# jzr99/Geo4D

Measured on AMD Instinct MI355X. Metric: denoised latent frames/sec (16x320x512, 50-step DDIM), higher is better.
Workload: dtype bf16x3m

## Files before the change

### geo4d_amd/_lib.py

```python
import ctypes as C
import os

import torch

_HERE = os.path.dirname(os.path.abspath(__file__))
LIB_PATH = os.environ.get("GEO4D_HIP_LIB") or os.path.join(_HERE, "csrc", "libgeo4d_hip.so")
ABI_VERSION = 9

F32, BF16, F16, BF16X3, F16X2 = 0, 1, 2, 3, 4


class Geo4DNativeError(RuntimeError):
    pass


class ConvGemm(C.Structure):
    _fields_ = [
        ("A", C.c_void_p), ("W", C.c_void_p), ("O", C.c_void_p),
        ("bias", C.c_void_p), ("rowbias", C.c_void_p), ("R", C.c_void_p),
        ("zeros", C.c_void_p), ("workspace", C.c_void_p), ("workspace_bytes", C.c_size_t),
        ("lda", C.c_long), ("ldw", C.c_long), ("ldo", C.c_long), ("ldr", C.c_long), ("ldrb", C.c_long),
        ("a_bs", C.c_long), ("w_bs", C.c_long), ("o_bs", C.c_long), ("r_bs", C.c_long),
        ("M", C.c_int), ("N", C.c_int), ("K", C.c_int), ("batch", C.c_int),
        ("Cin", C.c_int),
# ... 14 lines not shown
        ("ldx", C.c_long), ("ldy", C.c_long),
        ("F", C.c_int), ("HW", C.c_int), ("C", C.c_int), ("groups", C.c_int), ("frames_per_stat", C.c_int),
        ("act", C.c_int), ("dtype", C.c_int), ("eps", C.c_float), ("colsum", C.c_void_p), ("split_out", C.c_int), ("colsum_rows", C.c_int),
        ("sat_count", C.c_void_p),
    ]


class Attention(C.Structure):
    _fields_ = [
        ("q", C.c_void_p), ("o", C.c_void_p),
        ("k", C.c_void_p * 2), ("vt", C.c_void_p * 2), ("zeros", C.c_void_p),
        ("ldq", C.c_long), ("ldo", C.c_long), ("ldk", C.c_long * 2), ("ldvt", C.c_long * 2), ("vt_bs", C.c_long * 2),
        ("Nk", C.c_int * 2), ("kv_div", C.c_int * 2),
        ("B", C.c_int), ("H", C.c_int), ("Nq", C.c_int), ("nseg", C.c_int), ("head_dim", C.c_int), ("dtype", C.c_int),
        ("scale", C.c_float), ("split_out", C.c_int), ("variant", C.c_int), ("qkv_split", C.c_int),
    ]


class Align(C.Structure):
    _fields_ = [
        ("pred", C.c_void_p), ("conf", C.c_void_p), ("logdepth", C.c_void_p), ("cams", C.c_void_p), ("slot_trf", C.c_void_p),
        ("slot_ptr", C.c_void_p), ("slot_idx", C.c_void_p),
        ("grad_logdepth", C.c_void_p), ("img_sums", C.c_void_p), ("slot_sums", C.c_void_p),
        ("workspace", C.c_void_p), ("workspace_bytes", C.c_size_t),
        ("img_part", C.c_void_p), ("slot_part", C.c_void_p),
        ("invdepth", C.c_void_p), ("slot_st", C.c_void_p),
        ("n_imgs", C.c_int), ("n_slots", C.c_int), ("H", C.c_int), ("W", C.c_int), ("chunk_pixels", C.c_int), ("max_slots_per_image", C.c_int),
        ("conf_clamp", C.c_float), ("inv_area", C.c_float), ("depth_weight", C.c_float),
    ]


class AlignSmall(C.Structure):
    _fields_ = [
        ("im_poses", C.c_void_p), ("im_focals", C.c_void_p), ("pw_poses", C.c_void_p), ("cams", C.c_void_p), ("slot_trf", C.c_void_p),
        ("img_sums", C.c_void_p), ("slot_sums", C.c_void_p), ("group_ptr", C.c_void_p), ("group_entries", C.c_void_p), ("group_sums", C.c_void_p),
        ("scale_terms", C.c_void_p),
        ("grad_im_poses", C.c_void_p), ("grad_im_focals", C.c_void_p), ("grad_pw_poses", C.c_void_p), ("grad_s_depth", C.c_void_p),
        ("grad_t_depth", C.c_void_p), ("loss", C.c_void_p),
        ("slot_st", C.c_void_p), ("s_depth", C.c_void_p), ("t_depth", C.c_void_p), ("depth_ok", C.c_void_p),
        ("traj", C.c_void_p), ("traj_align", C.c_void_p), ("traj_valid", C.c_void_p), ("slot_img", C.c_void_p), ("img_slot_ptr", C.c_void_p),
        ("img_slot_idx", C.c_void_p), ("grad_traj", C.c_void_p),
        ("n_imgs", C.c_int), ("n_groups", C.c_int), ("n_slots", C.c_int), ("slots_per_group", C.c_int), ("n_listed_slots", C.c_int),
        ("n_focals", C.c_int), ("norm_pw_scale", C.c_int),
        ("focal_break", C.c_float), ("base_scale", C.c_float), ("ppx", C.c_float), ("ppy", C.c_float), ("smooth_weight", C.c_float),
        ("translation_weight", C.c_float), ("traj_weight", C.c_float),
    ]


SIGNATURES = {
    "geo4d_conv_gemm": (C.c_int, [C.POINTER(ConvGemm), C.c_void_p]),
    "geo4d_conv_gemm_colsum_rows": (C.c_int, [C.POINTER(ConvGemm)]),
    "geo4d_groupnorm_workspace": (C.c_size_t, [C.c_int, C.c_int, C.c_int, C.c_int]),
    "geo4d_groupnorm": (C.c_int, [C.POINTER(GroupNorm), C.c_void_p]),
    "geo4d_layernorm": (C.c_int, [C.c_void_p, C.c_long, C.c_void_p, C.c_long, C.c_int, C.c_int, C.c_float, C.c_void_p,
                                  C.c_void_p, C.c_int, C.c_void_p]),
    "geo4d_layernorm_split": (C.c_int, [C.c_void_p, C.c_long, C.c_void_p, C.c_long, C.c_int, C.c_int, C.c_float, C.c_void_p,
                                        C.c_void_p, C.c_int, C.c_void_p, C.c_void_p]),
    "geo4d_softmax_rows": (C.c_int, [C.c_void_p, C.c_long, C.c_void_p, C.c_long, C.c_long, C.c_int, C.c_float, C.c_int,
                                     C.c_void_p]),
    "geo4d_softmax_rows_causal": (C.c_int, [C.c_void_p, C.c_long, C.c_void_p, C.c_long, C.c_long, C.c_int, C.c_float, C.c_int,
                                            C.c_int, C.c_void_p]),
    "geo4d_attention": (C.c_int, [C.POINTER(Attention), C.c_void_p]),
    "geo4d_temporal_attention": (C.c_int, [C.c_void_p, C.c_long, C.c_void_p, C.c_long, C.c_void_p, C.c_long, C.c_void_p,
                                           C.c_long, C.c_int, C.c_int, C.c_int, C.c_int, C.c_int, C.c_float, C.c_int,
                                           C.c_void_p]),
    "geo4d_temporal_attention2": (C.c_int, [C.c_void_p, C.c_long, C.c_void_p, C.c_long, C.c_void_p, C.c_long, C.c_void_p,
                                            C.c_long, C.c_int, C.c_int, C.c_int, C.c_int, C.c_int, C.c_float, C.c_int,
                                            C.c_int, C.c_void_p]),
    "geo4d_tokens_from_ncthw": (C.c_int, [C.c_void_p, C.c_int, C.c_void_p, C.c_int, C.c_void_p, C.c_int, C.c_int, C.c_int,
                                          C.c_int, C.c_int, C.c_void_p]),
    "geo4d_cast_rows_f16": (C.c_int, [C.c_void_p, C.c_long, C.c_void_p, C.c_long, C.c_long, C.c_int, C.c_void_p, C.c_void_p]),
    "geo4d_split_rows_bf16": (C.c_int, [C.c_void_p, C.c_long, C.c_void_p, C.c_long, C.c_long, C.c_int, C.c_void_p]),
    "geo4d_concat_channels": (C.c_int, [C.c_void_p, C.c_long, C.c_int, C.c_void_p, C.c_long, C.c_int, C.c_void_p, C.c_long,
                                        C.c_long, C.c_int, C.c_void_p]),
    "geo4d_timestep_embedding": (C.c_int, [C.c_void_p, C.c_void_p, C.c_void_p, C.c_int, C.c_int, C.c_void_p]),
    "geo4d_linear_small": (C.c_int, [C.c_void_p, C.c_long, C.c_void_p, C.c_long, C.c_void_p, C.c_void_p, C.c_long,
                                     C.c_void_p, C.c_long, C.c_int, C.c_int, C.c_int, C.c_int, C.c_int, C.c_void_p]),
    "geo4d_ddim_step": (C.c_int, [C.c_void_p, C.c_void_p, C.c_void_p, C.c_void_p, C.c_void_p, C.c_void_p, C.c_long,
                                  C.c_void_p]),
    "geo4d_cfg_combine_workspace": (C.c_size_t, [C.c_int]),
    "geo4d_cfg_combine": (C.c_int, [C.c_void_p, C.c_void_p, C.c_void_p, C.c_void_p, C.c_int, C.c_long, C.c_float, C.c_float,
                                    C.c_float, C.c_void_p, C.c_size_t, C.c_void_p]),
    "geo4d_embed_tokens": (C.c_int, [C.c_void_p, C.c_void_p, C.c_void_p, C.c_void_p, C.c_long, C.c_long, C.c_int, C.c_int, C.c_int,
                                     C.c_int, C.c_void_p]),
    "geo4d_advance_index": (C.c_int, [C.c_void_p, C.c_int, C.c_void_p]),
    "geo4d_gather_timestep": (C.c_int, [C.c_void_p, C.c_void_p, C.c_void_p, C.c_int, C.c_void_p]),
    "geo4d_plucker_cameras_workspace": (C.c_size_t, [C.c_int, C.c_int, C.c_int]),
    "geo4d_plucker_cameras": (C.c_int, [C.c_void_p, C.c_void_p, C.c_long, C.c_long, C.c_int, C.c_int, C.c_int, C.c_void_p,
                                        C.c_size_t, C.c_void_p, C.c_void_p]),
    "geo4d_align_workspace": (C.c_size_t, [C.c_int, C.c_int, C.c_int, C.c_int, C.c_int]),
    "geo4d_align_residual": (C.c_int, [C.POINTER(Align), C.c_void_p]),
    "geo4d_adam_step": (C.c_int, [C.c_void_p, C.c_void_p, C.c_void_p, C.c_void_p, C.c_long, C.c_float, C.c_float, C.c_float, C.c_float,
                                  C.c_int, C.c_void_p]),
    "geo4d_adam_step_dev": (C.c_int, [C.c_void_p, C.c_void_p, C.c_void_p, C.c_void_p, C.c_long, C.c_void_p, C.c_float, C.c_float, C.c_float,
                                      C.c_void_p]),
    "geo4d_lad_workspace": (C.c_size_t, [C.c_int, C.c_long]),
    "geo4d_lad_target": (C.c_int, [C.c_void_p, C.c_void_p, C.c_void_p, C.c_int, C.c_int, C.c_void_p]),
    "geo4d_lower_median": (C.c_int, [C.c_void_p, C.c_int, C.c_long, C.c_void_p, C.c_void_p, C.c_size_t, C.c_void_p]),
    "geo4d_lad_fit": (C.c_int, [C.c_void_p, C.c_void_p, C.c_int, C.c_long, C.c_void_p, C.c_float, C.c_int, C.c_float, C.c_void_p, C.c_void_p,
                                C.c_void_p, C.c_size_t, C.c_void_p]),
    "geo4d_lad_delta": (C.c_int, [C.c_void_p, C.c_void_p, C.c_void_p, C.c_void_p, C.c_int, C.c_long, C.c_float, C.c_float, C.c_float,
                                  C.c_void_p, C.c_void_p]),
    "geo4d_bicubic_resize": (C.c_int, [C.c_void_p, C.c_void_p, C.c_int, C.c_int, C.c_int, C.c_int, C.c_int, C.c_void_p]),
    "geo4d_masked_select_workspace": (C.c_size_t, [C.c_long]),
    "geo4d_masked_select": (C.c_int, [C.c_void_p, C.c_void_p, C.c_long, C.c_float, C.c_void_p, C.c_float, C.c_float, C.c_void_p, C.c_void_p,
                                      C.c_void_p, C.c_void_p, C.c_size_t, C.c_void_p]),
# ... 56 lines not shown
```

### geo4d_amd/csrc/norm.hip

```cpp
#include <type_traits>
#include "common.h"
#include "geo4d_hip.h"

namespace {

__host__ __device__ inline int gn_rows_per_chunk(int HW, int F) {
    long r = ((long)HW * F + 1023) / 1024;
    r = (r + 3) / 4 * 4;
    if (r < 4) r = 4;
    if (r > 1024) r = 1024;
    return (int)r;
}

template <typename T>
__device__ __forceinline__ void gn_partial_body(char* smem, const T* __restrict__ x, long ldx, int HW, int C, int G,
                                                int R, int nchunk, float* __restrict__ part, int chunk, int f) {
    constexpr int EPC = Elem<T>::EPC;
    float* stage = (float*)smem;
    float* chs = stage + 256 * 2 * EPC;
    float* chq = chs + C;
    const int tid = threadIdx.x;
    const int CPR = C / EPC;
    const int TC = CPR < 256 ? CPR : 256;
    const int TR = 256 / TC;
// ... 50 lines not shown
        float m2 = qq - ss * mean;
        if (m2 < 0.f) m2 = 0.f;
        float* o = part + (((long)f * nchunk + chunk) * G + tid) * 3;
        o[0] = n; o[1] = mean; o[2] = m2;
    }
}
template <typename T>
__global__ __launch_bounds__(256) void gn_partial_kernel(const T* __restrict__ x, long ldx, int HW, int C, int G,
                                                         int R, int nchunk, float* __restrict__ part) {
    extern __shared__ __attribute__((aligned(16))) char smem[];
    gn_partial_body<T>(smem, x, ldx, HW, C, G, R, nchunk, part, blockIdx.x, blockIdx.y);
}

__device__ __forceinline__ void chan_merge(float& n, float& mean, float& m2, float nb, float mb, float qb) {
    if (nb > 0.f) {
        const float nn = n + nb;
        const float d = mb - mean;
        const float w = nb / nn;
        mean += d * w;
        m2 += qb + d * d * n * w;
        n = nn;
    }
}
__device__ __forceinline__ f32x2 gn_merge_unit(const float* __restrict__ part, int total, int stat, int grp, int G, float eps, int lane) {
    float n = 0.f, mean = 0.f, m2 = 0.f;
    for (int i = lane; i < total; i += 64) {
        const float* pp = part + (((long)stat * total + i) * G + grp) * 3;
        chan_merge(n, mean, m2, pp[0], pp[1], pp[2]);
    }
#pragma unroll
    for (int o = 1; o < 64; o <<= 1) {
        const float nb = __shfl_xor(n, o), mb = __shfl_xor(mean, o), qb = __shfl_xor(m2, o);
        float n0 = n, a0 = mean, q0 = m2, n1 = nb, a1 = mb, q1 = qb;
        if (lane & o) { n0 = nb; a0 = mb; q0 = qb; n1 = n; a1 = mean; q1 = m2; }
        chan_merge(n0, a0, q0, n1, a1, q1);
        n = n0; mean = a0; m2 = q0;
    }
    return f32x2{mean, 1.0f / sqrtf(m2 / n + eps)};
}
__global__ __launch_bounds__(256) void gn_finalize_kernel(const float* __restrict__ part, int nchunk, int fps, int G,
                                                          float eps, float* __restrict__ stats, int nstat) {
    const int lane = threadIdx.x & 63;
    const int unit = blockIdx.x * 4 + (threadIdx.x >> 6);
    if (unit >= nstat * G) return;
    const int stat = unit / G, grp = unit - stat * G;
    const f32x2 r = gn_merge_unit(part, fps * nchunk, stat, grp, G, eps, lane);
    if (lane == 0) {
        stats[((long)stat * G + grp) * 2 + 0] = r[0];
        stats[((long)stat * G + grp) * 2 + 1] = r[1];
    }
}

__global__ __launch_bounds__(256) void gn_finalize_cols_kernel(const float* __restrict__ colsum, int blocks_per_stat, int C, int G, float eps,
                                                               float* __restrict__ stats, int nstat, int rows) {
    __shared__ double red[4][2];
    const int tid = threadIdx.x, lane = tid & 63, wave = tid >> 6;
    const int unit = blockIdx.x;
    const int stat = unit / G, grp = unit - stat * G;
    const int cpg = C / G;
    double s = 0.0, q = 0.0;
    const int total = blocks_per_stat * cpg;
    for (int i = tid; i < total; i += 256) {
        const int rb = i / cpg, c = grp * cpg + (i - rb * cpg);
        const f32x2 sq = *(const f32x2*)(colsum + (((long)stat * blocks_per_stat + rb) * C + c) * 2);
        s += (double)sq[0];
        q += (double)sq[1];
    }
#pragma unroll
    for (int o = 1; o < 64; o <<= 1) {
        s += __shfl_xor(s, o);
        q += __shfl_xor(q, o);
    }
    if (lane == 0) { red[wave][0] = s; red[wave][1] = q; }
    __syncthreads();
    if (tid == 0) {
        s = ((red[0][0] + red[1][0]) + red[2][0]) + red[3][0];
        q = ((red[0][1] + red[1][1]) + red[2][1]) + red[3][1];
        const double n = (double)blocks_per_stat * rows * cpg;
        const double mean = s / n;
        double var = q / n - mean * mean;
        if (var < 0.0) var = 0.0;
        stats[((long)stat * G + grp) * 2 + 0] = (float)mean;
        stats[((long)stat * G + grp) * 2 + 1] = (float)(1.0 / sqrt(var + (double)eps));
    }
}

template <typename T, int SPLIT>
__device__ __forceinline__ void gn_apply_body(const T* __restrict__ x, long ldx, T* __restrict__ y, long ldy,
                                              int HW, int C, int G, int R, const float* st, const float* __restrict__ gamma,
                                              const float* __restrict__ beta, int act, int chunk, int f, unsigned long long* sat) {
    constexpr int EPC = Elem<T>::EPC;
    const int tid = threadIdx.x;
    const int CPR = C / EPC;
    const int TC = CPR < 256 ? CPR : 256;
    const int TR = 256 / TC;
    const int tc = tid % TC, tr = tid / TC;
    if (tr >= TR) return;
    const int row0 = chunk * R;
    const int rows = min(R, HW - row0);
    const int cpg = C / G;
    const T* xb = x + ((long)f * HW + row0) * ldx;
    T* yb = y + ((long)f * HW + row0) * ldy;
    for (int cc = tc; cc < CPR; cc += TC) {
        float sc[EPC], sh[EPC];
#pragma unroll
        for (int j = 0; j < EPC; ++j) {
            const int c = cc * EPC + j;
            const int gi = c / cpg;
            const float mean = st[gi * 2], rstd = st[gi * 2 + 1];
            sc[j] = rstd * gamma[c];
            sh[j] = beta[c] - mean * sc[j];
        }
        for (int r = tr; r < rows; r += 4 * TR) {
            u32x4 v[4];
#pragma unroll
            for (int u = 0; u < 4; ++u) {
                const int ru = r + u * TR;
// ... 105 lines not shown
        const u32x4 v = *(const u32x4*)(xr + (l + 16 * i) * 4);
#pragma unroll
        for (int j = 0; j < 4; ++j) { e[i][j] = __uint_as_float(v[j]); s += e[i][j]; }
    }
    const float mean = quarter_sum(s) / (float)C;
    float q = 0.f;
#pragma unroll
    for (int i = 0; i < NCH; ++i)
#pragma unroll
        for (int j = 0; j < 4; ++j) { const float d = e[i][j] - mean; q += d * d; }
    const float rstd = 1.0f / sqrtf(quarter_sum(q) / (float)C + eps);
    if (!ok) return;
#pragma unroll
    for (int i = 0; i < NCH; ++i) {
        const int cc = l + 16 * i;
        const f32x4 g = *(const f32x4*)(gamma + cc * 4), b = *(const f32x4*)(beta + cc * 4);
        float o[4];
#pragma unroll
        for (int j = 0; j < 4; ++j) o[j] = (e[i][j] - mean) * rstd * g[j] + b[j];
        if constexpr (SPLIT == 1) store_split4(y + row * ldy, cc, o);
        else if constexpr (SPLIT == 2) {
            count_f16_saturation(sat, o);
            store4_f16((char*)y + row * ldy * 2, cc, o);
        } else *(f32x4*)(y + row * ldy + cc * 4) = f32x4{o[0], o[1], o[2], o[3]};
    }
}

template <typename T>
__global__ __launch_bounds__(256) void softmax_rows_kernel(const float* __restrict__ x, long ldx, T* __restrict__ y, long ldy,
                                                           int cols_all, float scale, int causal_period) {
    __shared__ float red[4];
    const int tid = threadIdx.x;
    const float* xr = x + (long)blockIdx.x * ldx;
    T* yr = y + (long)blockIdx.x * ldy;
    const int cols = causal_period > 0 ? min(cols_all, (int)(blockIdx.x % causal_period) + 1) : cols_all;
    for (int c = cols + tid; c < cols_all; c += 256) Elem<T>::st(yr + c, 0.f);
    float m = -INFINITY;
    for (int c = tid; c < cols; c += 256) m = fmaxf(m, xr[c] * scale);
    m = wave_max(m);
    if ((tid & 63) == 0) red[tid >> 6] = m;
    __syncthreads();
    m = fmaxf(fmaxf(red[0], red[1]), fmaxf(red[2], red[3]));
    __syncthreads();
    float s = 0.f;
    for (int c = tid; c < cols; c += 256) s += __expf(xr[c] * scale - m);
    s = wave_sum(s);
    if ((tid & 63) == 0) red[tid >> 6] = s;
    __syncthreads();
    s = (red[0] + red[1]) + (red[2] + red[3]);
    const float inv = 1.0f / s;
    for (int c = tid; c < cols; c += 256) Elem<T>::st(yr + c, __expf(xr[c] * scale - m) * inv);
}

template <typename T, int SPLIT>
int groupnorm_typed(const geo4d_groupnorm_t& p, hipStream_t s) {
    constexpr int EPC = Elem<T>::EPC;
    int R = gn_rows_per_chunk(p.HW, p.F);
    int nchunk = (p.HW + R - 1) / R;
    float* part = (float*)p.workspace;
    const size_t smem = (size_t)256 * 2 * EPC * 4 + (size_t)2 * p.C * 4;
    const int nstat = p.F / p.frames_per_stat;
    float* stats = part + (size_t)p.F * nchunk * p.groups * 3;
    if (p.colsum) {
        const int crows = p.colsum_rows > 0 ? p.colsum_rows : 32;
        hipLaunchKernelGGL(gn_finalize_cols_kernel, dim3(nstat * p.groups), dim3(256), 0, s, p.colsum, (p.frames_per_stat * p.HW) / crows,
                           p.C, p.groups, p.eps, stats, nstat, crows);
        GEO4D_CHECK_LAUNCH();
    } else {
        hipLaunchKernelGGL(gn_partial_kernel<T>, dim3(nchunk, p.F), dim3(256), smem, s, (const T*)p.x, (long)p.ldx, p.HW, p.C, p.groups,
                           R, nchunk, part);
        GEO4D_CHECK_LAUNCH();
        hipLaunchKernelGGL(gn_finalize_kernel, dim3((nstat * p.groups + 3) / 4), dim3(256), 0, s, part, nchunk, p.frames_per_stat,
                           p.groups, p.eps, stats, nstat);
        GEO4D_CHECK_LAUNCH();
    }
    hipLaunchKernelGGL((gn_apply_kernel<T, SPLIT>), dim3(nchunk, p.F), dim3(256), 0, s, (const T*)p.x, (long)p.ldx, (T*)p.y, (long)p.ldy, p.HW,
                       p.C, p.groups, p.frames_per_stat, R, stats, p.gamma, p.beta, p.act, SPLIT == 2 ? p.sat_count : nullptr);
    GEO4D_CHECK_LAUNCH();
    return GEO4D_OK;
}

template <typename T, int SPLIT = 0>
int layernorm_typed(const void* x, long ldx, void* y, long ldy, int M, int C, float eps, const float* g, const float* b,
                    hipStream_t s, unsigned long long* sat = nullptr) {
    constexpr int EPC = Elem<T>::EPC;
    if constexpr (std::is_same<T, float>::value) {
        const bool al = ((uintptr_t)g % 16) == 0 && ((uintptr_t)b % 16) == 0;
        const dim3 grid16((M + 15) / 16);
#define LN16_LAUNCH(NC) hipLaunchKernelGGL((ln16_kernel<NC, SPLIT>), grid16, dim3(256), 0, s, (const float*)x, ldx, (float*)y, ldy, M, eps, g, b, sat)
        if (al && C == 320) { LN16_LAUNCH(5); GEO4D_CHECK_LAUNCH(); return GEO4D_OK; }
        if (al && C == 640) { LN16_LAUNCH(10); GEO4D_CHECK_LAUNCH(); return GEO4D_OK; }
#undef LN16_LAUNCH
    }
    const int per_lane = (C / EPC + 63) / 64;
    const dim3 grid((M + 3) / 4);
#define LN_LAUNCH(MC) hipLaunchKernelGGL((ln_kernel<T, MC, SPLIT>), grid, dim3(256), 0, s, (const T*)x, ldx, (T*)y, ldy, M, C, eps, g, b, sat)
    if (per_lane <= 1) LN_LAUNCH(1);
    else if (per_lane <= 2) LN_LAUNCH(2);
    else if (per_lane <= 3) LN_LAUNCH(3);
    else if (per_lane <= 5) LN_LAUNCH(5);
    else if (per_lane <= 10) LN_LAUNCH(10);
    else { geo4d_set_error("layernorm: C too large"); return GEO4D_ENOTSUP; }
#undef LN_LAUNCH
    GEO4D_CHECK_LAUNCH();
    return GEO4D_OK;
}

}

extern "C" size_t geo4d_groupnorm_workspace(int F, int HW, int groups, int frames_per_stat) {
    const int R = gn_rows_per_chunk(HW, F);
    const int nchunk = (HW + R - 1) / R;
    return ((size_t)F * nchunk * groups * 3 + (size_t)(F / frames_per_stat) * groups * 2) * sizeof(float);
}

extern "C" int geo4d_groupnorm(const geo4d_groupnorm_t* pp, void* stream) {
    if (!pp) return GEO4D_EINVAL;
    const geo4d_groupnorm_t& p = *pp;
    const int esz = p.dtype == GEO4D_F32 ? 4 : 2, epc = 16 / esz;
    if (p.dtype < 0 || p.dtype > 2) { geo4d_set_error("groupnorm: bad dtype"); return GEO4D_EINVAL; }
    if (p.F <= 0 || p.HW <= 0 || p.C <= 0 || p.groups <= 0 || p.groups > 32 || p.C % p.groups || p.C % epc) {
        geo4d_set_error("groupnorm: need C % groups == 0, C % (16 B) == 0, groups <= 32");
        return GEO4D_EINVAL;
    }
    if (p.frames_per_stat <= 0 || p.F % p.frames_per_stat) { geo4d_set_error("groupnorm: F % frames_per_stat"); return GEO4D_EINVAL; }
    const int yesz = p.split_out == 2 ? 2 : esz;
    if ((p.ldx * esz) % 16 || (p.ldy * yesz) % 16 || ((uintptr_t)p.x % 16) || ((uintptr_t)p.y % 16)) { geo4d_set_error("groupnorm: alignment"); return GEO4D_EINVAL; }
    if (p.workspace_bytes < geo4d_groupnorm_workspace(p.F, p.HW, p.groups, p.frames_per_stat)) { geo4d_set_error("groupnorm: workspace too small"); return GEO4D_EINVAL; }
    if (p.F > 65535) { geo4d_set_error("groupnorm: too many frames"); return GEO4D_EINVAL; }
    {
        const int crows = p.colsum_rows > 0 ? p.colsum_rows : 32;
        if (p.colsum && ((((long)p.frames_per_stat * p.HW) % crows) || ((uintptr_t)p.colsum % 8))) {
            geo4d_set_error("groupnorm: colsum needs (frames_per_stat x HW) % colsum_rows == 0");
            return GEO4D_EINVAL;
        }
    }
    if (p.split_out && (p.dtype != GEO4D_F32 || (p.C % 8) || p.split_out > 2 || p.split_out < 0)) { geo4d_set_error("groupnorm: split_out (1 = bf16 hi | lo, 2 = plain f16 rows) is a producer format for f32 input, C % 8 == 0"); return GEO4D_EINVAL; }
    hipStream_t s = (hipStream_t)stream;
    switch (p.dtype) {
        case GEO4D_F32: return p.split_out == 2 ? groupnorm_typed<float, 2>(p, s) : p.split_out ? groupnorm_typed<float, 1>(p, s) : groupnorm_typed<float, 0>(p, s);
        case GEO4D_BF16: return groupnorm_typed<bf16_t, 0>(p, s);
        default: return groupnorm_typed<f16_t, 0>(p, s);
    }
}

extern "C" int geo4d_layernorm(const void* x, long ldx, void* y, long ldy, int M, int C, float eps, const float* gamma,
                               const float* beta, int dtype, void* stream) {
    const int esz = dtype == GEO4D_F32 ? 4 : 2, epc = 16 / esz;
    if (dtype < 0 || dtype > 2 || M <= 0 || C <= 0 || C % epc || (ldx * esz) % 16 || (ldy * esz) % 16 || ((uintptr_t)x % 16) || ((uintptr_t)y % 16)) {
        geo4d_set_error("layernorm: bad arguments");
        return GEO4D_EINVAL;
    }
    hipStream_t s = (hipStream_t)stream;
    switch (dtype) {
        case GEO4D_F32: return layernorm_typed<float>(x, ldx, y, ldy, M, C, eps, gamma, beta, s);
        case GEO4D_BF16: return layernorm_typed<bf16_t>(x, ldx, y, ldy, M, C, eps, gamma, beta, s);
        default: return layernorm_typed<f16_t>(x, ldx, y, ldy, M, C, eps, gamma, beta, s);
    }
}

extern "C" int geo4d_layernorm_split(const void* x, long ldx, void* y, long ldy, int M, int C, float eps, const float* gamma,
                                     const float* beta, int fmt, unsigned long long* sat_count, void* stream) {
    if (M <= 0 || C <= 0 || C % 8 || (ldx * 4) % 16 || (ldy * (fmt == 2 ? 2 : 4)) % 16 || ((uintptr_t)x % 16) || ((uintptr_t)y % 16) || (fmt != 1 && fmt != 2)) {
        geo4d_set_error("layernorm_split: bad arguments (f32 input, C % 8 == 0, 16-byte aligned rows, fmt 1 = bf16 halves or 2 = plain f16 rows)");
        return GEO4D_EINVAL;
    }
    if (fmt == 2) return layernorm_typed<float, 2>(x, ldx, y, ldy, M, C, eps, gamma, beta, (hipStream_t)stream, sat_count);
    return layernorm_typed<float, 1>(x, ldx, y, ldy, M, C, eps, gamma, beta, (hipStream_t)stream);
}

static int softmax_rows_launch(const float* x, long ldx, void* y, long ldy, long rows, int cols, float scale, int out_dtype,
                               int causal_period, void* stream);
extern "C" int geo4d_softmax_rows(const float* x, long ldx, void* y, long ldy, long rows, int cols, float scale, int out_dtype,
                                  void* stream) {
    return softmax_rows_launch(x, ldx, y, ldy, rows, cols, scale, out_dtype, 0, stream);
}
extern "C" int geo4d_softmax_rows_causal(const float* x, long ldx, void* y, long ldy, long rows, int cols, float scale, int out_dtype,
                                         int causal_period, void* stream) {
    if (causal_period <= 0) { geo4d_set_error("softmax_rows_causal: causal_period must be positive"); return GEO4D_EINVAL; }
    return softmax_rows_launch(x, ldx, y, ldy, rows, cols, scale, out_dtype, causal_period, stream);
}
static int softmax_rows_launch(const float* x, long ldx, void* y, long ldy, long rows, int cols, float scale, int out_dtype,
                               int causal_period, void* stream) {
    if (rows <= 0 || cols <= 0 || out_dtype < 0 || out_dtype > 2 || rows > 2147483647L) { geo4d_set_error("softmax_rows: bad arguments"); return GEO4D_EINVAL; }
    hipStream_t s = (hipStream_t)stream;
    const dim3 grid((unsigned)rows);
    switch (out_dtype) {
        case GEO4D_F32: hipLaunchKernelGGL(softmax_rows_kernel<float>, grid, dim3(256), 0, s, x, ldx, (float*)y, ldy, cols, scale, causal_period); break;
        case GEO4D_BF16: hipLaunchKernelGGL(softmax_rows_kernel<bf16_t>, grid, dim3(256), 0, s, x, ldx, (bf16_t*)y, ldy, cols, scale, causal_period); break;
        default: hipLaunchKernelGGL(softmax_rows_kernel<f16_t>, grid, dim3(256), 0, s, x, ldx, (f16_t*)y, ldy, cols, scale, causal_period); break;
    }
    GEO4D_CHECK_LAUNCH();
    return GEO4D_OK;
}
```

### geo4d_amd/ops.py

```python
import ctypes as C

import torch

from . import _lib
from ._lib import BF16, BF16X3, F16, F16X2, F32, Attention, ConvGemm, GroupNorm
from .precision import resolve as _resolve_precision

_DT = {torch.float32: F32, torch.bfloat16: BF16, torch.float16: F16}
_TD = {F32: torch.float32, BF16: torch.bfloat16, F16: torch.float16}


def dt_code(dtype):
    try:
        return _DT[dtype]
    except KeyError:
        raise TypeError(f"geo4d_amd: unsupported dtype {dtype} (float32, bfloat16, float16 only)")


def k_align(dtype):
    return 32 if _resolve_precision(dtype).storage == torch.float32 else 64


class X2Weight(torch.Tensor):
    _KEEP = {"to", "clone", "detach", "contiguous", "cuda", "cpu", "pin_memory"}
# ... 359 lines not shown
            out = torch.empty((M, N), device=x.device, dtype=_out_dtype(x, out_dtype, w))
    conv_gemm(x, w, out, M=M, N=N, K=KH * KW * Cin, Cin=Cin, lda=_ld(x), ldw=_ld(w), ldo=(nchw_channels or N) if out_nchw else _ld(out), T=T,
              Hin=Hin, Win=Win, Hout=Hout, Wout=Wout, KH=KH, KW=KW, ph=pad, pw=pad, stride=stride, ups=ups, bias=bias,
              rowbias=rowbias, rowbias_div=rowbias_div, residual=residual,
              ldr=_ld(residual) if residual is not None else 0, act=act, out_nchw=out_nchw, tile_hint=tile_hint,
              split_k=split_k, gn_stats=gn_stats)
    return out, Hout, Wout


def conv_temporal(x, w, bias, *, B, T, HW, residual=None, out=None, gn_stats=False, tile_hint=0, split_k=0):
    Cin = act_k(x)
    N = w.shape[0]
    M = B * T * HW
    assert x.shape[0] == M and kdim(w, x) == 3 * Cin
    if out is None:
        out = torch.empty((M, N), device=x.device, dtype=_out_dtype(x, None, w))
    return conv_gemm(x, w, out, M=M, N=N, K=3 * Cin, Cin=Cin, lda=_ld(x), ldw=_ld(w), ldo=_ld(out), T=T, Hin=HW, Win=1,
                     Hout=HW, Wout=1, KT=3, pt=1, bias=bias, residual=residual,
                     ldr=_ld(residual) if residual is not None else 0, gn_stats=gn_stats, tile_hint=tile_hint, split_k=split_k)


def batched_gemm(a, b, out, *, batch, M, N, K, a_bs, b_bs, o_bs, bias=None, bias_per_row=False, alpha=1.0, x3=False):
    return conv_gemm(a, b, out, M=M, N=N, K=K, Cin=K, lda=_ld(a), ldw=_ld(b), ldo=_ld(out), batch=batch, a_bs=a_bs,
                     w_bs=b_bs, o_bs=o_bs, bias=bias, bias_per_row=bias_per_row, alpha=alpha, x3=x3)


_gn_ws = {}


def groupnorm(x, gamma, beta, *, F, HW, eps, groups=32, frames_per_stat=1, silu=False, out=None, split_out=False):
    lib = _lib.load()
    _dev(x, "x")
    assert not isinstance(x, SplitAct), "GroupNorm reads plain activations"
    Cc = x.shape[1]
    assert x.shape[0] == F * HW, (x.shape, F, HW)
    assert gamma.dtype == torch.float32 and beta.dtype == torch.float32
    if out is None:
        out = new_split(F * HW, Cc, x.device, split_fmt(split_out)[1]) if split_out else torch.empty((F * HW, Cc), device=x.device, dtype=x.dtype)
    split_out = 1 if isinstance(out, SplitAct) else 2 if (out.dtype == torch.float16 and x.dtype == torch.float32) else 0
    if split_out:
        assert x.dtype == torch.float32, "the GEMM-operand producer formats are written from f32 activations"
    if split_out == 1:
        _split_out_ok(out, F * HW)
    need = lib.geo4d_groupnorm_workspace(F, HW, groups, frames_per_stat)
    ws = torch.empty(need, device=x.device, dtype=torch.uint8)
    p = GroupNorm()
    p.x, p.y, p.gamma, p.beta = x.data_ptr(), out.data_ptr(), gamma.data_ptr(), beta.data_ptr()
    p.workspace, p.workspace_bytes = ws.data_ptr(), need
    p.ldx, p.ldy = _ld(x), (_ld(out) // 2 if split_out == 1 else _ld(out))
    p.split_out = int(split_out)
    p.sat_count = _ptr(SAT_COUNTER) if split_out == 2 else 0
    p.F, p.HW, p.C, p.groups, p.frames_per_stat = F, HW, Cc, groups, frames_per_stat
    p.act, p.dtype, p.eps = int(silu), dt_code(x.dtype), eps
    cs = getattr(x, "_gn_colsum", None)
    if cs is not None and getattr(x, "_gn_colsum_tag", None) != (x.data_ptr(), x._version):
        cs = None
    rows = getattr(x, "_gn_colsum_rows", 32)
    ok = cs is not None and (frames_per_stat * HW) % rows == 0 and tuple(cs.shape) == (F * HW // rows, Cc, 2)
    p.colsum, p.colsum_rows = (cs.data_ptr(), rows) if ok else (0, 0)
    _lib.check(lib.geo4d_groupnorm(C.byref(p), _stream()), "geo4d_groupnorm")
    return out


def layernorm(x, gamma, beta, eps=1e-5, out=None, split_out=False):
    lib = _lib.load()
    _dev(x, "x")
    assert not isinstance(x, SplitAct), "LayerNorm reads plain activations"
    M, Cc = x.shape
    if split_out or isinstance(out, SplitAct) or (out is not None and out.dtype == torch.float16 and x.dtype == torch.float32):
        assert x.dtype == torch.float32
        if out is None:
            out = new_split(M, Cc, x.device, split_fmt(split_out)[1])
        if isinstance(out, SplitAct):
            _split_out_ok(out, M)
            _lib.check(lib.geo4d_layernorm_split(x.data_ptr(), _ld(x), out.data_ptr(), _ld(out) // 2, M, Cc, eps, gamma.data_ptr(),
                                                 beta.data_ptr(), 1, 0, _stream()), "geo4d_layernorm_split")
        else:
            assert out.dtype == torch.float16
            _lib.check(lib.geo4d_layernorm_split(x.data_ptr(), _ld(x), out.data_ptr(), _ld(out), M, Cc, eps, gamma.data_ptr(),
                                                 beta.data_ptr(), 2, _ptr(SAT_COUNTER), _stream()), "geo4d_layernorm_split")
        return out
    if out is None:
        out = torch.empty((M, Cc), device=x.device, dtype=x.dtype)
    _lib.check(lib.geo4d_layernorm(x.data_ptr(), _ld(x), out.data_ptr(), _ld(out), M, Cc, eps, gamma.data_ptr(),
                                   beta.data_ptr(), dt_code(x.dtype), _stream()), "geo4d_layernorm")
    return out


def softmax_rows(x, scale, out_dtype, out=None, causal_period=0):
    lib = _lib.load()
    _dev(x, "x")
    assert x.dtype == torch.float32
    rows, cols = x.shape
    if out is None:
        out = torch.empty((rows, cols), device=x.device, dtype=out_dtype)
    if causal_period:
        _lib.check(lib.geo4d_softmax_rows_causal(x.data_ptr(), _ld(x), out.data_ptr(), _ld(out), rows, cols, scale,
                                                 dt_code(out.dtype), causal_period, _stream()), "geo4d_softmax_rows_causal")
    else:
        _lib.check(lib.geo4d_softmax_rows(x.data_ptr(), _ld(x), out.data_ptr(), _ld(out), rows, cols, scale,
                                          dt_code(out.dtype), _stream()), "geo4d_softmax_rows")
    return out


ATTN_VARIANT = int(_os.environ.get("GEO4D_ATTN_VARIANT", "0"))


def attention(q, kv, *, B, H, Nq, scale, out=None, x3=False, variant=None, split_out=False, qkv_split=False):
    lib = _lib.load()
    if qkv_split:
        assert len(kv) == 1 and all(isinstance(t, SplitAct) for t in (q, kv[0][0], kv[0][1])), "qkv_split takes SplitAct q / k / vt of one key/value set"
        return _attention_presplit(lib, q, kv[0], B=B, H=H, Nq=Nq, scale=scale, out=out, variant=variant, split_out=split_out)
    _dev(q, "q")
    if out is None:
# ... 385 lines not shown
```

### geo4d_amd/unet.py

```python
import math
import os

import torch
import torch.nn as nn

from . import ops, pack
from .precision import resolve as resolve_dtype


class ParamTree(nn.Module):

    def __init__(self):
        super().__init__()

    def insert(self, dotted, shape):
        node = self
        parts = dotted.split(".")
        for part in parts[:-1]:
            child = node._modules.get(part)
            if child is None:
                child = ParamTree()
                node.add_module(part, child)
            node = child
        node.register_parameter(parts[-1], nn.Parameter(torch.empty(shape), requires_grad=False))
# ... 419 lines not shown
            n1 = ops.layernorm(x, *blk["norm1"], split_out=sp)
            qk = ops.linear(n1, blk["attn1.qk"])
            vt, npad = ops.linear_t_batched(blk["attn1.v"], n1, F_, N)
            att = ops.attention(qk[:, :C_], [(qk[:, C_:], vt.reshape(-1, npad), N, 1, C_ * npad)], B=F_, H=heads, Nq=N, scale=0.125, x3=x3, split_out=sp)
        x = ops.linear(att, *blk["attn1.o"], residual=x)
        c16 = blk.get("x2cattn")
        q = ops.linear(ops.layernorm(x, *blk["norm2"], split_out="f16" if blk.get("x2ln") else sp), blk["attn2.q"], split_out="f16" if c16 else False)
        k_t, k_i, vt_t, vt_i, _, h16 = kv
        off, _ = e["kv"]
        if c16:
            sets = [(h16["k_t"][:, off:off + C_], h16["vt_t." + L.prefix].reshape(-1, 80), 77, T, C_ * 80)]
            if k_i is not None:
                sets.append((h16["k_i"][:, off:off + C_], h16["vt_i." + L.prefix], 16, 1, 16))
            att = ops.attention(q, sets, B=F_, H=heads, Nq=N, scale=0.125)
        else:
            sets = [(k_t[:, off:off + C_], vt_t[L.prefix].reshape(-1, 80), 77, T, C_ * 80)]
            if k_i is not None:
                sets.append((k_i[:, off:off + C_], vt_i[L.prefix], 16, 1, 16))
            att = ops.attention(q, sets, B=F_, H=heads, Nq=N, scale=0.125, x3=x3, split_out=sp)
        x = ops.linear(att, *blk["attn2.o"], residual=x)
        x = self._ff(blk, x)
        return ops.linear(x, *e["out"], residual=h, gn_stats=True, out=out)

    def _temporal(self, e, L, h, B, T, H, W, out=None):
        F_, HW, C_, heads = B * T, H * W, L.inner, L.heads
        blk = e["blk"]
        sp = self.presplit
        x = ops.linear(ops.groupnorm(h, *e["norm"], F=F_, HW=HW, eps=1e-6, frames_per_stat=T, split_out="f16" if e.get("x2in") else sp), *e["in"])
        t16 = blk.get("x2tattn")
        for a, n in (("attn1", "norm1"), ("attn2", "norm2")):
            qkv = ops.linear(ops.layernorm(x, *blk[n], split_out="f16" if blk.get("x2ln") else sp), blk[a + ".qkv"], split_out="f16" if t16 else False)
            att = ops.temporal_attention(qkv[:, :C_], qkv[:, C_:2 * C_], qkv[:, 2 * C_:], B=B, T=T, HW=HW, H=heads, scale=0.125, split_out=False if t16 else sp)
            x = ops.linear(att, *blk[a + ".o"], residual=x)
        x = self._ff(blk, x)
        return ops.linear(x, *e["out"], residual=h, gn_stats=True, out=out)

    def _run(self, P, layers, h, emb_all, kv, B, T, H, W, out=None):
        for L in layers:
            e = P[L.prefix]
            o = None
            if out is not None and L is layers[-1]:
                Ho, Wo = ((H - 1) // 2 + 1, (W - 1) // 2 + 1) if L.kind == "down" else (2 * H, 2 * W) if L.kind == "up" else (H, W)
                o = out(B * T * Ho * Wo)
            if L.kind == "res":
                h = self._res(e, L, h, emb_all, B, T, H, W, out=o)
            elif L.kind == "spatial":
                h = self._spatial(e, L, h, kv, B, T, H, W, out=o)
            elif L.kind == "temporal":
                h = self._temporal(e, L, h, B, T, H, W, out=o)
            elif L.kind == "down":
                h, H, W = ops.conv2d(h, e["w"], e["b"], F=B * T, Hin=H, Win=W, KH=3, KW=3, stride=2, pad=1, gn_stats=True, out=o)
            elif L.kind == "up":
                a = ops.presplit(h) if (self.presplit and PRESPLIT_UP) else h
                h, H, W = ops.conv2d(a, e["w"], e["b"], F=B * T, Hin=H, Win=W, KH=3, KW=3, pad=1, ups=2, out=o)
        return h, H, W

    @torch.no_grad()
    def forward(self, x, timesteps, context=None, features_adapter=None, fs=None, task=None, c_concat=None, **kwargs):
        if features_adapter is not None or task is not None:
            raise NotImplementedError("features_adapter / task conditioning are not part of Geo4D inference")
        if timesteps.dim() != 1:
            raise NotImplementedError("per-frame timesteps (2-D) have no HIP path")
        P = self._packed or self._pack()
        B, C0, T, H, W = x.shape
        C1 = 0 if c_concat is None else c_concat.shape[1]
        assert C0 + C1 == self.in_channels, f"expected {self.in_channels} input channels, got {C0}+{C1}"
        if T > 16:
            raise NotImplementedError("temporal_length > 16 has no HIP path (configs/inference_geo4d.yaml:89)")
        dt = self.storage_dtype
        inputs, middle, outputs, init_attn, _ = self.layout
        t_emb = ops.timestep_embedding(timesteps.to(torch.int64), P["freqs"])
        w0, b0, w2, b2 = P["time"]
        emb = ops.linear_small(ops.linear_small(t_emb, w0, b0, act_out=True), w2, b2)
        if self.fs_condition:
            if fs is None:
                fs = torch.full((B,), self.default_fs, dtype=torch.int64, device=x.device)
            w0, b0, w2, b2 = P["fps"]
            f_emb = ops.timestep_embedding(fs.to(torch.int64), P["freqs"])
            emb = ops.linear_small(ops.linear_small(f_emb, w0, b0, act_out=True), w2, b2, add=emb)
        emb_all = ops.linear_small(emb, P["emb_w"], P["emb_b"], act_in=True)
        kv = self._context_kv(P, context, B, T)
        e0 = P[inputs[0][0].prefix]
        h = ops.tokens_from_ncthw(x.float().contiguous(), None if c_concat is None else c_concat.float().contiguous(), e0["cpad"], dt)
        n_in = len(inputs)
        cats = {}

        def half(j, left):
            if not FUSED_CONCAT or j >= len(outputs):
                return None
            ccat = outputs[j][0].cin

            def view(rows, j=j, left=left, ccat=ccat):
                buf = cats.get(j)
                if buf is None:
                    buf = cats[j] = torch.empty((rows, ccat), device=x.device, dtype=dt)
                assert buf.shape[0] == rows, "latent height/width must be multiples of 8"
                cs = skip_ch[n_in - 1 - j]
                return buf[:, :ccat - cs] if left else buf[:, ccat - cs:]
            return view
        skip_ch = [blk[-1].cout if blk[-1].kind != "temporal" and blk[-1].kind != "spatial" else blk[-1].cin for blk in inputs]
        o0 = half(n_in - 1, False)
        if init_attn is not None:
            h, _, _ = ops.conv2d(h, e0["w"], e0["b"], F=B * T, Hin=H, Win=W, KH=3, KW=3, pad=1, gn_stats=True)
            h = self._temporal(P[init_attn.prefix], init_attn, h, B, T, H, W, out=None if o0 is None else o0(B * T * H * W))
        else:
            h, _, _ = ops.conv2d(h, e0["w"], e0["b"], F=B * T, Hin=H, Win=W, KH=3, KW=3, pad=1, gn_stats=True, out=None if o0 is None else o0(B * T * H * W))
        hs = [(h, H, W)]
        for i, blk in enumerate(inputs[1:], start=1):
            h, H, W = self._run(P, blk, h, emb_all, kv, B, T, H, W, out=half(n_in - 1 - i, False))
            hs.append((h, H, W))
        h, H, W = self._run(P, middle, h, emb_all, kv, B, T, H, W, out=half(0, True))
        for j, blk in enumerate(outputs):
            s, sh, sw = hs.pop()
            assert (sh, sw) == (H, W), "latent height/width must be multiples of 8"
            hc = cats.pop(j) if j in cats else ops.concat_channels(h, s)
            h, H, W = self._run(P, blk, hc, emb_all, kv, B, T, H, W, out=half(j + 1, True))
        a = ops.groupnorm(h, *P["out_gn"], F=B * T, HW=H * W, eps=1e-5, silu=True, split_out=self.presplit)
        y, _, _ = ops.conv2d(a, P["out_w"], P["out_b"], F=B * T, Hin=H, Win=W, KH=3, KW=3, pad=1, T=T, out_nchw=True,
                             out_dtype=torch.float32)
        return y if x.dtype == torch.float32 else y.to(x.dtype)
```

### include/geo4d_hip.h

```cpp
#ifndef GEO4D_HIP_H
#define GEO4D_HIP_H
#include <stddef.h>
#ifdef __cplusplus
extern "C" {
#endif

#define GEO4D_ABI_VERSION 9

typedef struct geo4d_conv_gemm_t {
    const void* A;
    const void* W;
    void* O;
    const float* bias;
    const float* rowbias;
    const void* R;
    const void* zeros;
    void* workspace;
    size_t workspace_bytes;
    long lda, ldw, ldo, ldr;
    long ldrb;
    long a_bs, w_bs, o_bs, r_bs;
    int M, N, K, batch;
    int Cin;
    int T, Hin, Win, Hout, Wout;
    int KT, KH, KW, pt, ph, pw, stride, ups;
    int rowbias_div;
    int bias_per_row;
    int act;
    int dtype;
    int out_dtype;
    int out_nchw;
    int tile_hint;
    int split_k;
    int debug_ablate;
    float alpha;
    int a_split, w_split;
    int o_split;
    float* gn_colsum;
    unsigned long long* sat_count;
} geo4d_conv_gemm_t;
int geo4d_conv_gemm(const geo4d_conv_gemm_t* p, void* stream);
int geo4d_conv_gemm_colsum_rows(const geo4d_conv_gemm_t* p);

typedef struct geo4d_groupnorm_t {
    const void* x; void* y;
    const float* gamma; const float* beta;
    void* workspace; size_t workspace_bytes;
    long ldx, ldy;
    int F, HW, C, groups, frames_per_stat;
    int act;
    int dtype;
    float eps;
    const float* colsum;
    int split_out;
    int colsum_rows;
    unsigned long long* sat_count;
} geo4d_groupnorm_t;
size_t geo4d_groupnorm_workspace(int F, int HW, int groups, int frames_per_stat);
int geo4d_groupnorm(const geo4d_groupnorm_t* p, void* stream);

int geo4d_layernorm(const void* x, long ldx, void* y, long ldy, int M, int C, float eps, const float* gamma,
                    const float* beta, int dtype, void* stream);

int geo4d_layernorm_split(const void* x, long ldx, void* y, long ldy, int M, int C, float eps, const float* gamma,
                          const float* beta, int fmt, unsigned long long* sat_count, void* stream);

int geo4d_softmax_rows(const float* x, long ldx, void* y, long ldy, long rows, int cols, float scale, int out_dtype,
                       void* stream);
int geo4d_softmax_rows_causal(const float* x, long ldx, void* y, long ldy, long rows, int cols, float scale, int out_dtype,
                              int causal_period, void* stream);

typedef struct geo4d_attention_t {
    const void* q; void* o;
    const void* k[2]; const void* vt[2];
    const void* zeros;
    long ldq, ldo, ldk[2], ldvt[2], vt_bs[2];
    int Nk[2], kv_div[2];
    int B, H, Nq, nseg, head_dim, dtype;
    float scale;
    int split_out;
    int variant;
    int qkv_split;
} geo4d_attention_t;
int geo4d_attention(const geo4d_attention_t* p, void* stream);

int geo4d_temporal_attention(const void* q, long ldq, const void* k, long ldk, const void* v, long ldv, void* o, long ldo,
                             int B, int T, int HW, int H, int head_dim, float scale, int dtype, void* stream);
int geo4d_temporal_attention2(const void* q, long ldq, const void* k, long ldk, const void* v, long ldv, void* o, long ldo,
                              int B, int T, int HW, int H, int head_dim, float scale, int dtype, int split_out, void* stream);

int geo4d_tokens_from_ncthw(const float* src0, int C0, const float* src1, int C1, void* out, int Cpad, int B, int T, int HW,
                            int dtype, void* stream);

int geo4d_concat_channels(const void* a, long lda, int Ca, const void* b, long ldb, int Cb, void* out, long ldo, long M,
                          int dtype, void* stream);

int geo4d_cast_rows_f16(const float* x, long ldx, void* y, long ldy, long M, int C, unsigned long long* sat_count, void* stream);

int geo4d_split_rows_bf16(const float* x, long ldx, void* y, long ldy, long M, int C, void* stream);

int geo4d_timestep_embedding(const long* t, const float* freqs, float* out, int B, int dim, void* stream);

int geo4d_linear_small(const float* x, long ldx, const float* w, long ldw, const float* bias, const float* add, long ldadd,
                       float* out, long ldo, int M, int N, int K, int act_in, int act_out, void* stream);

int geo4d_ddim_step(float* x, const float* v, const float* noise, float* pred_x0, const float* coef, const int* step_index,
                    long n, void* stream);
size_t geo4d_cfg_combine_workspace(int B);
int geo4d_cfg_combine(const float* e_c, const float* e_u, const float* e_i, float* out, int B, long n, float scale, float cfg_img,
                      float guidance_rescale, void* workspace, size_t workspace_bytes, void* stream);
int geo4d_embed_tokens(const long* tokens, const float* table, const float* pos, void* out, long ldo, long rows, int n_ctx,
                       int width, int vocab, int dtype, void* stream);
// ... 80 lines not shown
```

Baseline: 6.772.

## Reuse producer column sums for groupnorm over fused channel-concat buffers

When the decoder's skip concat is written in place by two producers (the left and right halves of a shared buffer), groupnorm now merges the per-column sum and sum-of-squares that each producer's GEMM epilogue already emitted. This replaces a separate statistics pass over the whole concatenated tensor. The upsample conv now also emits gn_stats so its half carries column sums. The cost is extra epilogue work in the up conv, plus bookkeeping that tracks views and checks their pointers.

```diff
diff --git a/geo4d_amd/_lib.py b/geo4d_amd/_lib.py
--- a/geo4d_amd/_lib.py
+++ b/geo4d_amd/_lib.py
@@ -90,6 +90,7 @@
     "geo4d_conv_gemm_colsum_rows": (C.c_int, [C.POINTER(ConvGemm)]),
     "geo4d_groupnorm_workspace": (C.c_size_t, [C.c_int, C.c_int, C.c_int, C.c_int]),
     "geo4d_groupnorm": (C.c_int, [C.POINTER(GroupNorm), C.c_void_p]),
+    "geo4d_groupnorm_concat": (C.c_int, [C.POINTER(GroupNorm), C.c_void_p, C.c_int, C.c_int, C.c_void_p]),
     "geo4d_layernorm": (C.c_int, [C.c_void_p, C.c_long, C.c_void_p, C.c_long, C.c_int, C.c_int, C.c_float, C.c_void_p,
                                   C.c_void_p, C.c_int, C.c_void_p]),
     "geo4d_layernorm_split": (C.c_int, [C.c_void_p, C.c_long, C.c_void_p, C.c_long, C.c_int, C.c_int, C.c_float, C.c_void_p,
diff --git a/geo4d_amd/csrc/norm.hip b/geo4d_amd/csrc/norm.hip
--- a/geo4d_amd/csrc/norm.hip
+++ b/geo4d_amd/csrc/norm.hip
@@ -126,17 +126,28 @@
 }
 
 __global__ __launch_bounds__(256) void gn_finalize_cols_kernel(const float* __restrict__ colsum, int blocks_per_stat, int C, int G, float eps,
-                                                               float* __restrict__ stats, int nstat, int rows) {
+                                                               float* __restrict__ stats, int nstat, int rows, int Ca,
+                                                               const float* __restrict__ colsum_b, int blocks_per_stat_b) {
     __shared__ double red[4][2];
     const int tid = threadIdx.x, lane = tid & 63, wave = tid >> 6;
     const int unit = blockIdx.x;
     const int stat = unit / G, grp = unit - stat * G;
     const int cpg = C / G;
     double s = 0.0, q = 0.0;
-    const int total = blocks_per_stat * cpg;
+    const int c0 = grp * cpg;
+    const int na = min(max(Ca - c0, 0), cpg);
+    const int nb = cpg - na;
+    const int total = blocks_per_stat * na;
     for (int i = tid; i < total; i += 256) {
-        const int rb = i / cpg, c = grp * cpg + (i - rb * cpg);
-        const f32x2 sq = *(const f32x2*)(colsum + (((long)stat * blocks_per_stat + rb) * C + c) * 2);
+        const int rb = i / na, c = c0 + (i - rb * na);
+        const f32x2 sq = *(const f32x2*)(colsum + (((long)stat * blocks_per_stat + rb) * Ca + c) * 2);
+        s += (double)sq[0];
+        q += (double)sq[1];
+    }
+    const int total_b = blocks_per_stat_b * nb, Cb = C - Ca;
+    for (int i = tid; i < total_b; i += 256) {
+        const int rb = i / nb, c = c0 + na - Ca + (i - rb * nb);
+        const f32x2 sq = *(const f32x2*)(colsum_b + (((long)stat * blocks_per_stat_b + rb) * Cb + c) * 2);
         s += (double)sq[0];
         q += (double)sq[1];
     }
@@ -348,8 +359,10 @@
     for (int c = tid; c < cols; c += 256) Elem<T>::st(yr + c, __expf(xr[c] * scale - m) * inv);
 }
 
+struct ColsumB { const float* colsum; int rows, c_split; };
+
 template <typename T, int SPLIT>
-int groupnorm_typed(const geo4d_groupnorm_t& p, hipStream_t s) {
+int groupnorm_typed(const geo4d_groupnorm_t& p, const ColsumB& cb, hipStream_t s) {
     constexpr int EPC = Elem<T>::EPC;
     int R = gn_rows_per_chunk(p.HW, p.F);
     int nchunk = (p.HW + R - 1) / R;
@@ -359,8 +372,9 @@
     float* stats = part + (size_t)p.F * nchunk * p.groups * 3;
     if (p.colsum) {
         const int crows = p.colsum_rows > 0 ? p.colsum_rows : 32;
-        hipLaunchKernelGGL(gn_finalize_cols_kernel, dim3(nstat * p.groups), dim3(256), 0, s, p.colsum, (p.frames_per_stat * p.HW) / crows,
-                           p.C, p.groups, p.eps, stats, nstat, crows);
+        const int span = p.frames_per_stat * p.HW;
+        hipLaunchKernelGGL(gn_finalize_cols_kernel, dim3(nstat * p.groups), dim3(256), 0, s, p.colsum, span / crows, p.C, p.groups, p.eps, stats, nstat, crows,
+                           cb.colsum ? cb.c_split : p.C, cb.colsum, cb.colsum ? span / cb.rows : 0);
         GEO4D_CHECK_LAUNCH();
     } else {
         hipLaunchKernelGGL(gn_partial_kernel<T>, dim3(nchunk, p.F), dim3(256), smem, s, (const T*)p.x, (long)p.ldx, p.HW, p.C, p.groups,
@@ -410,7 +424,7 @@
     return ((size_t)F * nchunk * groups * 3 + (size_t)(F / frames_per_stat) * groups * 2) * sizeof(float);
 }
 
-extern "C" int geo4d_groupnorm(const geo4d_groupnorm_t* pp, void* stream) {
+static int groupnorm_launch(const geo4d_groupnorm_t* pp, const ColsumB& cb, void* stream) {
     if (!pp) return GEO4D_EINVAL;
     const geo4d_groupnorm_t& p = *pp;
     const int esz = p.dtype == GEO4D_F32 ? 4 : 2, epc = 16 / esz;
@@ -434,10 +448,22 @@
     if (p.split_out && (p.dtype != GEO4D_F32 || (p.C % 8) || p.split_out > 2 || p.split_out < 0)) { geo4d_set_error("groupnorm: split_out (1 = bf16 hi | lo, 2 = plain f16 rows) is a producer format for f32 input, C % 8 == 0"); return GEO4D_EINVAL; }
     hipStream_t s = (hipStream_t)stream;
     switch (p.dtype) {
-        case GEO4D_F32: return p.split_out == 2 ? groupnorm_typed<float, 2>(p, s) : p.split_out ? groupnorm_typed<float, 1>(p, s) : groupnorm_typed<float, 0>(p, s);
-        case GEO4D_BF16: return groupnorm_typed<bf16_t, 0>(p, s);
-        default: return groupnorm_typed<f16_t, 0>(p, s);
-    }
+        case GEO4D_F32: return p.split_out == 2 ? groupnorm_typed<float, 2>(p, cb, s) : p.split_out ? groupnorm_typed<float, 1>(p, cb, s) : groupnorm_typed<float, 0>(p, cb, s);
+        case GEO4D_BF16: return groupnorm_typed<bf16_t, 0>(p, cb, s);
+        default: return groupnorm_typed<f16_t, 0>(p, cb, s);
+    }
+}
+
+extern "C" int geo4d_groupnorm(const geo4d_groupnorm_t* pp, void* stream) { return groupnorm_launch(pp, ColsumB{nullptr, 0, 0}, stream); }
+
+extern "C" int geo4d_groupnorm_concat(const geo4d_groupnorm_t* pp, const float* colsum_b, int colsum_b_rows, int c_split, void* stream) {
+    if (!pp) return GEO4D_EINVAL;
+    if (!pp->colsum || !colsum_b || colsum_b_rows <= 0 || c_split <= 0 || c_split >= pp->C || ((uintptr_t)colsum_b % 8) || pp->frames_per_stat <= 0 ||
+        (((long)pp->frames_per_stat * pp->HW) % colsum_b_rows)) {
+        geo4d_set_error("groupnorm_concat: needs both producers' column sums, 0 < c_split < C and (frames_per_stat x HW) % rows == 0 for either");
+        return GEO4D_EINVAL;
+    }
+    return groupnorm_launch(pp, ColsumB{colsum_b, colsum_b_rows, c_split}, stream);
 }
 
 extern "C" int geo4d_layernorm(const void* x, long ldx, void* y, long ldy, int M, int C, float eps, const float* gamma,
diff --git a/geo4d_amd/ops.py b/geo4d_amd/ops.py
--- a/geo4d_amd/ops.py
+++ b/geo4d_amd/ops.py
@@ -435,14 +435,32 @@
     p.sat_count = _ptr(SAT_COUNTER) if split_out == 2 else 0
     p.F, p.HW, p.C, p.groups, p.frames_per_stat = F, HW, Cc, groups, frames_per_stat
     p.act, p.dtype, p.eps = int(silu), dt_code(x.dtype), eps
-    cs = getattr(x, "_gn_colsum", None)
-    if cs is not None and getattr(x, "_gn_colsum_tag", None) != (x.data_ptr(), x._version):
-        cs = None
-    rows = getattr(x, "_gn_colsum_rows", 32)
-    ok = cs is not None and (frames_per_stat * HW) % rows == 0 and tuple(cs.shape) == (F * HW // rows, Cc, 2)
-    p.colsum, p.colsum_rows = (cs.data_ptr(), rows) if ok else (0, 0)
+    def sums_of(t, width):
+        cs = getattr(t, "_gn_colsum", None)
+        if cs is None or getattr(t, "_gn_colsum_tag", None) != (t.data_ptr(), t._version):
+            return None
+        rows = getattr(t, "_gn_colsum_rows", 32)
+        return (cs, rows) if (frames_per_stat * HW) % rows == 0 and tuple(cs.shape) == (F * HW // rows, width, 2) else None
+
+    parts = getattr(x, "_gn_concat_parts", None)
+    if parts is not None:
+        left, right = parts
+        ca = left.shape[1]
+        a = sums_of(left, ca) if (left.data_ptr() == x.data_ptr() and right.data_ptr() == x.data_ptr() + ca * x.element_size() and ca + right.shape[1] == Cc) else None
+        b = sums_of(right, Cc - ca) if a is not None else None
+        if b is not None:
+            p.colsum, p.colsum_rows = a[0].data_ptr(), a[1]
+            _lib.check(lib.geo4d_groupnorm_concat(C.byref(p), b[0].data_ptr(), b[1], ca, _stream()), "geo4d_groupnorm_concat")
+            return out
+    own = sums_of(x, Cc)
+    p.colsum, p.colsum_rows = (own[0].data_ptr(), own[1]) if own is not None else (0, 0)
     _lib.check(lib.geo4d_groupnorm(C.byref(p), _stream()), "geo4d_groupnorm")
     return out
+
+
+def concat_parts(buf, left, right):
+    buf._gn_concat_parts = (left, right)
+    return buf
 
 
 def layernorm(x, gamma, beta, eps=1e-5, out=None, split_out=False):
diff --git a/geo4d_amd/unet.py b/geo4d_amd/unet.py
--- a/geo4d_amd/unet.py
+++ b/geo4d_amd/unet.py
@@ -495,7 +495,7 @@
                 h, H, W = ops.conv2d(h, e["w"], e["b"], F=B * T, Hin=H, Win=W, KH=3, KW=3, stride=2, pad=1, gn_stats=True, out=o)
             elif L.kind == "up":
                 a = ops.presplit(h) if (self.presplit and PRESPLIT_UP) else h
-                h, H, W = ops.conv2d(a, e["w"], e["b"], F=B * T, Hin=H, Win=W, KH=3, KW=3, pad=1, ups=2, out=o)
+                h, H, W = ops.conv2d(a, e["w"], e["b"], F=B * T, Hin=H, Win=W, KH=3, KW=3, pad=1, ups=2, gn_stats=True, out=o)
         return h, H, W
 
     @torch.no_grad()
@@ -527,6 +527,7 @@
         h = ops.tokens_from_ncthw(x.float().contiguous(), None if c_concat is None else c_concat.float().contiguous(), e0["cpad"], dt)
         n_in = len(inputs)
         cats = {}
+        views = {}
 
         def half(j, left):
             if not FUSED_CONCAT or j >= len(outputs):
@@ -539,7 +540,8 @@
                     buf = cats[j] = torch.empty((rows, ccat), device=x.device, dtype=dt)
                 assert buf.shape[0] == rows, "latent height/width must be multiples of 8"
                 cs = skip_ch[n_in - 1 - j]
-                return buf[:, :ccat - cs] if left else buf[:, ccat - cs:]
+                v = views[(j, left)] = buf[:, :ccat - cs] if left else buf[:, ccat - cs:]
+                return v
             return view
         skip_ch = [blk[-1].cout if blk[-1].kind != "temporal" and blk[-1].kind != "spatial" else blk[-1].cin for blk in inputs]
         o0 = half(n_in - 1, False)
@@ -556,7 +558,7 @@
         for j, blk in enumerate(outputs):
             s, sh, sw = hs.pop()
             assert (sh, sw) == (H, W), "latent height/width must be multiples of 8"
-            hc = cats.pop(j) if j in cats else ops.concat_channels(h, s)
+            hc = ops.concat_parts(cats.pop(j), views[(j, True)], views[(j, False)]) if j in cats else ops.concat_channels(h, s)
             h, H, W = self._run(P, blk, hc, emb_all, kv, B, T, H, W, out=half(j + 1, True))
         a = ops.groupnorm(h, *P["out_gn"], F=B * T, HW=H * W, eps=1e-5, silu=True, split_out=self.presplit)
         y, _, _ = ops.conv2d(a, P["out_w"], P["out_b"], F=B * T, Hin=H, Win=W, KH=3, KW=3, pad=1, T=T, out_nchw=True,
diff --git a/include/geo4d_hip.h b/include/geo4d_hip.h
--- a/include/geo4d_hip.h
+++ b/include/geo4d_hip.h
@@ -58,6 +58,7 @@
 } geo4d_groupnorm_t;
 size_t geo4d_groupnorm_workspace(int F, int HW, int groups, int frames_per_stat);
 int geo4d_groupnorm(const geo4d_groupnorm_t* p, void* stream);
+int geo4d_groupnorm_concat(const geo4d_groupnorm_t* p, const float* colsum_b, int colsum_b_rows, int c_split, void* stream);
 
 int geo4d_layernorm(const void* x, long ldx, void* y, long ldy, int M, int C, float eps, const float* gamma,
                     const float* beta, int dtype, void* stream);
```

Result: no change. 6.783, median of 6 (+0.2%).
